# Avielstein/GRASP_LAB_SALP

Hardware: AMD Instinct MI355X
Metric: env-steps/sec at 65536 parallel envs, 1/2/4/8 MI355X; % HBM roofline (higher is better)
Workload: dtype f64

## Files before the change

grasp_lab_salp_amd/csrc/salp_device.h:

```cpp
#ifndef SALP_DEVICE_H
#define SALP_DEVICE_H

#include <hip/hip_runtime.h>
#include <stdint.h>

#include "../../include/salp.h"
#include "salp_math.h"
#include "salp_philox.h"
#include "salp_random.h"

#pragma clang fp contract(off)

static_assert(SALP_FMA, "libsalp.so is built in the product arithmetic mode (salp_math.h)");

#define SD static __device__ __forceinline__
#define SD_MEMBER __device__ __forceinline__
#define SD_HOST_DEV static __host__ __device__ __forceinline__

namespace salp {

constexpr double DT = 0.01;
constexpr double PI = 3.141592653589793;
constexpr double COS_GAMMA = 0x1.6a09e667f3bcdp-1;
constexpr double SIN_GAMMA = 0x1.6a09e667f3bccp-1;
// ... 765 lines not shown
        SF(SALP_F_AMF0 + j) = k.amf[j]; SF(SALP_F_AMRF0 + j) = k.amrf[j];
        SF(SALP_F_AMT0 + j) = k.amt[j]; SF(SALP_F_AMRT0 + j) = k.amrt[j];
    }
    h.rnd.cd = k.cd; h.rnd.dfr = k.dfr; h.rnd.dtr = k.dtr;
    h.rnd.amf0 = k.amf[0]; h.rnd.amf1 = k.amf[1]; h.rnd.amf2 = k.amf[2];
    h.rnd.amrf0 = k.amrf[0]; h.rnd.amrf1 = k.amrf[1]; h.rnd.amrf2 = k.amrf[2];
    h.rnd.amt0 = k.amt[0]; h.rnd.amt1 = k.amt[1]; h.rnd.amt2 = k.amt[2];
}

template <bool RAND = false, class ST>
SD void set_control(Hot& h, ST S, const Params& P, int64_t i, double contraction, double coast,
                    double a1, double a2, bool c32, const double* dir = nullptr) {
    set_coefficients<RAND>(h, S, P, i);
    SF(SALP_F_AVGV0) = 0.0; SF(SALP_F_AVGV1) = 0.0; SF(SALP_F_AVGV2) = 0.0;
    SF(SALP_F_AVGW0) = 0.0; SF(SALP_F_AVGW1) = 0.0; SF(SALP_F_AVGW2) = 0.0;
    h.c = contraction;
    h.coast = coast;
    h.c32 = c32;
    h.turn = nozzle_set_angles(S, P, i, a1, a2);
    if (dir) {
        h.d0 = dir[0]; h.d1 = dir[1]; h.d2 = dir[2];
    } else {
        nozzle_direction(a1, a2, &h.d0);
    }
    SF(SALP_F_CYCLE) = SF(SALP_F_CYCLE) + 1.0;
    h.ct = 0.0;
    const double sq = c32 ? (double)sqf((float)h.c) : h.c * h.c;
    h.refill = REFILL_C0 * sq + REFILL_C1 * h.c + REFILL_C2;
    h.jet = PROPUL_C0 * sq + PROPUL_C1 * h.c + PROPUL_C2;
    h.cr = h.refill > 0 ? h.c / h.refill : 0.0;
    h.rr = h.jet > 0 ? h.c / h.jet : 0.0;
    cycle_bounds(h);
}

template <class ST>
SD void cycle_prologue(const Hot& h, ST S, const Params& P, int64_t i) {
    const double total = h.b2;
    double pq0 = SF(SALP_F_PPOS0), pq1 = SF(SALP_F_PPOS1), pq2 = SF(SALP_F_PPOS2);
    double pg0 = SF(SALP_F_PANG0), pg1 = SF(SALP_F_PANG1), pg2 = SF(SALP_F_PANG2);
    SF(SALP_F_AVGV0) = (h.q0 - pq0) / total; SF(SALP_F_AVGV1) = (h.q1 - pq1) / total;
    SF(SALP_F_AVGV2) = (h.q2 - pq2) / total;
    SF(SALP_F_AVGW0) = (h.g0 - pg0) / total; SF(SALP_F_AVGW1) = (h.g1 - pg1) / total;
    SF(SALP_F_AVGW2) = (h.g2 - pg2) / total;
    SF(SALP_F_PPOS0) = h.q0; SF(SALP_F_PPOS1) = h.q1; SF(SALP_F_PPOS2) = h.q2;
    SF(SALP_F_PANG0) = h.g0; SF(SALP_F_PANG1) = h.g1; SF(SALP_F_PANG2) = h.g2;
    SF(SALP_F_PENDING) = 1.0;
}

struct StepPlan {
    float a0, a1, a2;
    double an1, an2;
    double d[3];
};
SD StepPlan plan_step(const Params& P, float a0, float a1, float a2, Cache32 c32) {
    StepPlan p;
    p.a0 = a0; p.a1 = a1; p.a2 = a2;
    const float r0 = a0 * 0.06f, r2 = a2 * (float)(PI / 2);
    nozzle_ik((double)r2, true, &p.an1, &p.an2);
    nozzle_direction(p.an1, p.an2, p.d);
    fill_cache32(P, (double)r0, c32);
    return p;
}
template <class ST>
SD void apply_step(Hot& h, ST S, const Params& P, int64_t i, const StepPlan& p) {
    SF(SALP_F_ACT0) = p.a0; SF(SALP_F_ACT1) = p.a1; SF(SALP_F_ACT2) = p.a2;
    const float r0 = p.a0 * 0.06f, r1 = p.a1 * 10.0f, r2 = p.a2 * (float)(PI / 2);
    SF(SALP_F_PREV_YAW) = SF(SALP_F_YAW);
    SF(SALP_F_YAW) = (double)r2;
    SF(SALP_F_PREV_ANGLE1) = SF(SALP_F_ANGLE1);
    SF(SALP_F_PREV_ANGLE2) = SF(SALP_F_ANGLE2);
    SF(SALP_F_ANGLE1) = p.an1;
    SF(SALP_F_ANGLE2) = p.an2;
    set_control<false>(h, S, P, i, (double)r0, (double)r1, p.an1, p.an2, true, p.d);
    cycle_prologue(h, S, P, i);
}

template <bool RAND = false, class ST>
SD void begin_step(Hot& h, ST S, const Params& P, int64_t i, float a0, float a1, float a2,
                   Cache32 c32) {
    SF(SALP_F_ACT0) = a0; SF(SALP_F_ACT1) = a1; SF(SALP_F_ACT2) = a2;
    float r0 = a0 * 0.06f, r1 = a1 * 10.0f, r2 = a2 * (float)(PI / 2);
    if (RAND && P.rand_act) {
        const float rr[3] = {r0, r1, r2};
        double ra[3];
        sr_randomize_action(P.seed, h.env_id, (uint64_t)SF(SALP_F_STEP_COUNT), rr, ra);
        nozzle_solve(S, P, i, ra[2], false);
        set_control<RAND>(h, S, P, i, ra[0], ra[1], SF(SALP_F_ANGLE1), SF(SALP_F_ANGLE2), false);
    } else {
        nozzle_solve(S, P, i, (double)r2, true);
        set_control<RAND>(h, S, P, i, (double)r0, (double)r1, SF(SALP_F_ANGLE1), SF(SALP_F_ANGLE2), true);
    }
    fill_cache32(P, h.c, c32);
    cycle_prologue(h, S, P, i);
}

template <class ST>
SD void record_state(const Hot& h, const Params& P, ST S, int64_t i, double* rec,
                     int64_t rs, bool first) {
    auto put = [&](int col, double x) { rec[(int64_t)col * rs] = x; };
    put(SALP_T_STATE, (double)h.phase);
    put(SALP_T_PW0, h.p0); put(SALP_T_PW1, h.p1); put(SALP_T_PW2, h.p2);
    put(SALP_T_V0, h.v0); put(SALP_T_V1, h.v1); put(SALP_T_V2, h.v2);
    put(SALP_T_ACC0, h.a0); put(SALP_T_ACC1, h.a1); put(SALP_T_ACC2, h.a2);
    put(SALP_T_ETA0, h.e0); put(SALP_T_ETA1, h.e1); put(SALP_T_ETA2, h.e2);
    put(SALP_T_W0, h.w0); put(SALP_T_W1, h.w1); put(SALP_T_W2, h.w2);
    put(SALP_T_ALPHA0, h.al0); put(SALP_T_ALPHA1, h.al1); put(SALP_T_ALPHA2, h.al2);
    put(SALP_T_LENGTH, h.L); put(SALP_T_WIDTH, h.W);
    const Core c = core(h.L, h.W, h.g32);
    const Shape sh = shape_of(P, c, h.L, h.W, h.g32);
    put(SALP_T_AREA0, sh.A0); put(SALP_T_AREA1, sh.A1); put(SALP_T_AREA2, sh.A1);
    put(SALP_T_VOLUME, h.V);
    put(SALP_T_MASS, h.geo.m);
    put(SALP_T_MASS_RATE, h.geo.mr);
    put(SALP_T_I0, h.geo.I0); put(SALP_T_I1, h.geo.I1); put(SALP_T_I2, h.geo.I1);
// ... 113 lines not shown
    bool done = false, trunc = false;
    if (dist < 0.2) { done = true; reward += 500.0; }
    else if (dist > 5.0) { trunc = true; reward -= 200.0; }
    if (hit) { trunc = true; reward -= 200.0; }
    if (SF(SALP_F_CYCLE) >= (double)P.max_cycles) { trunc = true; reward -= 50.0; }
    const double nlen = ep_len + 1.0;
    SF(SALP_F_EP_LEN) = nlen;
    const double ret = SF(SALP_F_EP_RETURN) + reward;
    SF(SALP_F_EP_RETURN) = ret;
    const double sa0 = SF(SALP_F_SUM_A0) + (double)(float)SF(SALP_F_ACT0);
    const double sa1 = SF(SALP_F_SUM_A1) + (double)(float)SF(SALP_F_ACT1);
    const double sa2 = SF(SALP_F_SUM_ABS_A2) + (double)fabsf(a2);
    SF(SALP_F_SUM_A0) = sa0; SF(SALP_F_SUM_A1) = sa1; SF(SALP_F_SUM_ABS_A2) = sa2;
    double sr[7];
#pragma unroll
    for (int k = 0; k < 7; ++k) {
        sr[k] = SF(SALP_F_SUM_R0 + k) + comp[k];
        SF(SALP_F_SUM_R0 + k) = sr[k];
    }
    if (info) {
        for (int k = 0; k < SALP_INFO_DIM; ++k) info[k] = 0.0;
        for (int k = 0; k < 7; ++k) info[SALP_INFO_R_TRACK + k] = comp[k];
        info[SALP_INFO_EP_RETURN] = ret;
        info[SALP_INFO_EP_LEN] = nlen;
        info[SALP_INFO_HIT_OBSTACLE] = hit ? 1.0 : 0.0;
        if (done || trunc) {
            double dd = np_norm2(px - 0.0, py - 0.0);
            info[SALP_INFO_HAS_METRICS] = 1.0;
            info[SALP_INFO_PATH_LENGTH] = path;
            info[SALP_INFO_DIRECT_DISTANCE] = dd;
            info[SALP_INFO_PATH_EFFICIENCY] = path > 0 ? dd / path : 0.0;
            info[SALP_INFO_FINAL_DISTANCE] = dist;
            info[SALP_INFO_INITIAL_DISTANCE] = SF(SALP_F_INIT_DIST);
            info[SALP_INFO_AVG_COMPRESSION] = sa0 / nlen;
            info[SALP_INFO_AVG_COAST_TIME] = sa1 / nlen;
            info[SALP_INFO_AVG_NOZZLE_ANGLE] = sa2 / nlen;
            info[SALP_INFO_AVG_VELOCITY] = svel / (nlen + 1.0);
            for (int k = 0; k < 7; ++k) info[SALP_INFO_AVG_R_TRACK + k] = sr[k] / nlen;
        }
    }
    SF(SALP_F_PREV_A2) = (double)a2;
    SF(SALP_F_PENDING) = 0.0;
    if (RAND && P.latency) {
        const double lat = sr_latency(P.seed, h.env_id, (uint64_t)SF(SALP_F_STEP_COUNT));
        set_control<RAND>(h, S, P, i, 0.0, lat, SF(SALP_F_ANGLE1), SF(SALP_F_ANGLE2), false);
    }
    out.reward = reward;
    out.terminated = done;
    out.truncated = trunc;
    out.hit = hit;
    return out;
}

SD int draw_reset(const Params& P, uint64_t env_id, uint64_t episode, float* tgt, float* obst) {
    double u0, u1;
    sp_reset_pair(P.seed, env_id, episode, 0u, &u0, &u1);
    double tx = P.x_min + (P.x_max - P.x_min) * u0, ty = P.y_min + (P.y_max - P.y_min) * u1;
    if (tx < P.x_min) tx = P.x_min;
    if (tx > P.x_max) tx = P.x_max;
    if (ty < P.y_min) ty = P.y_min;
    if (ty > P.y_max) ty = P.y_max;
    tgt[0] = (float)tx; tgt[1] = (float)ty;
    int n = 0;
    for (int k = 0; k < P.num_obstacles; ++k) {
        for (int att = 0; att < 200; ++att) {
            sp_reset_pair(P.seed, env_id, episode, (uint32_t)(1 + k * 200 + att), &u0, &u1);
            float px = (float)(P.x_min + (P.x_max - P.x_min) * u0);
            float py = (float)(P.y_min + (P.y_max - P.y_min) * u1);
            float ds = sqrtf(sm_fmaf(py, py, px * px));
            float ex = px - tgt[0], ey = py - tgt[1];
            float dtg = sqrtf(sm_fmaf(ey, ey, ex * ex));
            bool close = false;
            for (int j = 0; j < n; ++j) {
                float fx = px - obst[2 * j], fy = py - obst[2 * j + 1];
                if ((double)sqrtf(sm_fmaf(fy, fy, fx * fx)) < P.sep) close = true;
            }
            if ((double)ds > 0.5 && (double)dtg > 0.5 && !close) {
                obst[2 * n] = px; obst[2 * n + 1] = py; ++n;
                break;
            }
        }
    }
    return n;
}

template <class ST>
SD void robot_reset(Hot& h, ST S, const Params& P, int64_t i) {
    h.time = 0.0; h.ct = 0.0; h.phase = REST;
    SF(SALP_F_CYCLE) = 0.0;
    h.v0 = h.v1 = h.v2 = 0.0; h.w0 = h.w1 = h.w2 = 0.0;
    h.a0 = h.a1 = h.a2 = 0.0; h.al0 = h.al1 = h.al2 = 0.0;
    h.e0 = h.e1 = h.e2 = 0.0; h.p0 = h.p1 = h.p2 = 0.0;
    h.q0 = h.q1 = h.q2 = 0.0; h.g0 = h.g1 = h.g2 = 0.0;
    SF(SALP_F_PPOS0) = 0.0; SF(SALP_F_PPOS1) = 0.0; SF(SALP_F_PPOS2) = 0.0;
    SF(SALP_F_PANG0) = 0.0; SF(SALP_F_PANG1) = 0.0; SF(SALP_F_PANG2) = 0.0;
    {
        const Core old = core(h.L, h.W, h.g32);
        h.com = center_of_mass(P, old, water_mass(P, h.V, h.g32), h.g32);
    }
    h.comr = (h.com - h.com) / DT;
    h.coma = (h.comr - h.comr) / DT;
    h.L = P.L0; h.W = P.W0; h.g32 = false;
    const Core c0 = core(h.L, h.W, false);
    h.V = water_volume(P, c0, false);
    h.pV = h.V; h.pv32 = false;
    refresh_derived(h, P);
    h.pI0 = h.geo.I0; h.pI1 = h.geo.I1; h.pI2 = h.geo.I1;
    if (P.rand_dist) {
        SF(SALP_F_OUF0) = 0.0; SF(SALP_F_OUF1) = 0.0; SF(SALP_F_OUF2) = 0.0;
        SF(SALP_F_OUT0) = 0.0; SF(SALP_F_OUT1) = 0.0; SF(SALP_F_OUT2) = 0.0;
        h.rnd.ouf0 = 0.0; h.rnd.ouf1 = 0.0; h.rnd.out2 = 0.0;
    }
    SF(SALP_F_PENDING) = 0.0;
}

template <class ST>
SD void reset_env(Hot& h, ST S, const Params& P, int64_t i, const float* tgt,
                  const float* obst, int nob, float* obs) {
    SF(SALP_F_TARGET0) = tgt[0]; SF(SALP_F_TARGET1) = tgt[1];
#pragma unroll
    for (int k = 0; k < SALP_MAX_OBSTACLES; ++k) {
        SF(SALP_F_OBST0 + 2 * k) = k < nob ? (double)obst[2 * k] : 0.0;
        SF(SALP_F_OBST0 + 2 * k + 1) = k < nob ? (double)obst[2 * k + 1] : 0.0;
    }
    SF(SALP_F_N_OBST) = nob;
    robot_reset(h, S, P, i);
    const double d0 = h.p0 - (double)tgt[0], d1 = h.p1 - (double)tgt[1];
    const double dist = np_norm2(d0, d1);
    SF(SALP_F_PREV_DIST) = dist;
    SF(SALP_F_PREV_A2) = 0.0;
    SF(SALP_F_ACT0) = 0.0; SF(SALP_F_ACT1) = 0.0; SF(SALP_F_ACT2) = 0.0;
    SF(SALP_F_EP_LEN) = 0.0; SF(SALP_F_EP_RETURN) = 0.0; SF(SALP_F_PATH_LEN) = 0.0;
    SF(SALP_F_LAST_PX) = h.p0; SF(SALP_F_LAST_PY) = h.p1;
    SF(SALP_F_SUM_A0) = 0.0; SF(SALP_F_SUM_A1) = 0.0; SF(SALP_F_SUM_ABS_A2) = 0.0;
    SF(SALP_F_SUM_VEL) = np_norm2(0.0, 0.0);
    SF(SALP_F_INIT_DIST) = dist;
#pragma unroll
    for (int k = 0; k < 7; ++k) SF(SALP_F_SUM_R0 + k) = 0.0;
    SF(SALP_F_EPISODE) = SF(SALP_F_EPISODE) + 1.0;
    SF(SALP_F_PENDING) = 0.0;
    if (obs) {
        Rot R = rot_zyx(h.e0, h.e1, h.e2);
        observation(h, R, S, P, i, obs);
    }
}

template <class ST>
SD void reset_env_philox(Hot& h, ST S, const Params& P, int64_t i, float* obs) {
    float tgt[2], obst[2 * SALP_MAX_OBSTACLES];
    int nob = draw_reset(P, (uint64_t)(P.env_offset + i), (uint64_t)SF(SALP_F_EPISODE), tgt, obst);
    reset_env(h, S, P, i, tgt, obst, nob, obs);
}

template <bool RAND>
SD void load_cold(ColdRegs<RAND>& C, double* S, const Params& P, int64_t i) {
    C.g = S + i;
    C.n = P.n;
    if (!SALP_COLD_BLOCK) {
#pragma unroll
        for (int f = 0; f < SALP_NUM_FIELDS; ++f)
            if (is_cached<RAND>(f)) C.v[f] = S[(size_t)f * (size_t)P.n + (size_t)i];
        return;
    }
    const double2* blk = reinterpret_cast<const double2*>(S + P.cold_off + (size_t)i * COLD_SLOTS);
    double v[kLayout.n_cold + 1];
#pragma unroll
    for (int k = 0; k < (kLayout.n_cold + 1) / 2; ++k) {
        const double2 x = blk[k];
        v[2 * k] = x.x;
        v[2 * k + 1] = x.y;
    }
#pragma unroll
    for (int f = 0; f < SALP_NUM_FIELDS; ++f) {
        if (kLayout.slot[f] >= 0) C.v[f] = v[kLayout.slot[f]];
        else if (is_cached<RAND>(f)) C.v[f] = S[(size_t)kLayout.row[f] * (size_t)P.n + (size_t)i];
    }
}
template <bool RAND>
SD void store_cold(const ColdRegs<RAND>& C, double* S, const Params& P, int64_t i) {
    if (!SALP_COLD_BLOCK) {
#pragma unroll
        for (int f = 0; f < SALP_NUM_FIELDS; ++f)
            if (is_cached<RAND>(f)) S[(size_t)f * (size_t)P.n + (size_t)i] = C.v[f];
        return;
    }
    double v[kLayout.n_cold + 1];
#pragma unroll
    for (int f = 0; f < SALP_NUM_FIELDS; ++f) {
        if (kLayout.slot[f] >= 0) v[kLayout.slot[f]] = C.v[f];
        else if (is_cached<RAND>(f)) S[(size_t)kLayout.row[f] * (size_t)P.n + (size_t)i] = C.v[f];
    }
    v[kLayout.n_cold] = 0.0;
    double2* blk = reinterpret_cast<double2*>(S + P.cold_off + (size_t)i * COLD_SLOTS);
#pragma unroll
    for (int k = 0; k < (kLayout.n_cold + 1) / 2; ++k) blk[k] = make_double2(v[2 * k], v[2 * k + 1]);
}

constexpr int SPILL_N = 63;
constexpr int SPILL_D0 = 43;
struct SpillSlot {
    double* p;
    int stride = LANES;
    SD_MEMBER double& operator[](int k) const { return p[k * stride]; }
};
template <bool RAND>
SD void spill(const Hot& h, SpillSlot s) {
    const Hot::Rnd& r = h.rnd;
    const double v[SPILL_N] = {
        h.v0, h.v1, h.v2, h.w0, h.w1, h.w2, h.a0, h.a1, h.a2, h.al0, h.al1, h.al2,
        h.e0, h.e1, h.e2, h.p0, h.p1, h.p2, h.q0, h.q1, h.q2, h.g0, h.g1, h.g2,
        h.L, h.W, h.V, h.pV, h.com, h.comr, h.coma, h.pI0, h.pI1, h.pI2, h.ct, h.time,
        h.refill, h.jet, h.coast, h.c, h.cr, h.rr, h.turn, h.d0, h.d1, h.d2,
        (double)(h.phase | (h.g32 ? 4 : 0) | (h.pv32 ? 8 : 0) | (h.c32 ? 16 : 0)),
        RAND ? r.cd : h.sp, RAND ? r.dfr : h.cp, RAND ? r.dtr : h.st, RAND ? r.amf0 : h.cth,
        RAND ? r.amf1 : h.geo.m, RAND ? r.amf2 : h.geo.mr, RAND ? r.amrf0 : h.geo.I0,
        RAND ? r.amrf1 : h.geo.I1, RAND ? r.amrf2 : h.geo.kc0, RAND ? r.amt0 : h.geo.kc1,
        RAND ? r.amt1 : h.geo.ra0, RAND ? r.amt2 : h.geo.ra1, RAND ? r.ouf0 : h.geo.dimx,
        RAND ? r.ouf1 : h.geo.dimy, RAND ? r.out2 : h.geo.speed, RAND ? r.tick : h.geo.rx};
#pragma unroll
    for (int k = 0; k < SPILL_N; ++k) s[k] = v[k];
}
template <bool RAND>
SD void unspill(Hot& h, SpillSlot s, const Params& P, uint64_t env_id) {
    double v[SPILL_N];
#pragma unroll
    for (int k = 0; k < SPILL_N; ++k) v[k] = s[k];
    h.v0 = v[0]; h.v1 = v[1]; h.v2 = v[2]; h.w0 = v[3]; h.w1 = v[4]; h.w2 = v[5];
    h.a0 = v[6]; h.a1 = v[7]; h.a2 = v[8]; h.al0 = v[9]; h.al1 = v[10]; h.al2 = v[11];
    h.e0 = v[12]; h.e1 = v[13]; h.e2 = v[14]; h.p0 = v[15]; h.p1 = v[16]; h.p2 = v[17];
    h.q0 = v[18]; h.q1 = v[19]; h.q2 = v[20]; h.g0 = v[21]; h.g1 = v[22]; h.g2 = v[23];
    h.L = v[24]; h.W = v[25]; h.V = v[26]; h.pV = v[27]; h.com = v[28]; h.comr = v[29]; h.coma = v[30];
    h.pI0 = v[31]; h.pI1 = v[32]; h.pI2 = v[33]; h.ct = v[34]; h.time = v[35];
    h.refill = v[36]; h.jet = v[37]; h.coast = v[38]; h.c = v[39]; h.cr = v[40]; h.rr = v[41];
    h.turn = v[42]; h.d0 = v[43]; h.d1 = v[44]; h.d2 = v[45];
    const int fl = (int)v[46];
    h.phase = fl & 3; h.g32 = (fl & 4) != 0; h.pv32 = (fl & 8) != 0; h.c32 = (fl & 16) != 0;
    h.env_id = env_id;
    if (RAND) {
        Hot::Rnd& r = h.rnd;
        r.cd = v[47]; r.dfr = v[48]; r.dtr = v[49]; r.amf0 = v[50]; r.amf1 = v[51]; r.amf2 = v[52];
        r.amrf0 = v[53]; r.amrf1 = v[54]; r.amrf2 = v[55]; r.amt0 = v[56]; r.amt1 = v[57];
        r.amt2 = v[58]; r.ouf0 = v[59]; r.ouf1 = v[60]; r.out2 = v[61]; r.tick = v[62];
        refresh_derived(h, P);
    } else {
        h.sp = v[47]; h.cp = v[48]; h.st = v[49]; h.cth = v[50];
        h.geo.m = v[51]; h.geo.mr = v[52]; h.geo.I0 = v[53]; h.geo.I1 = v[54]; h.geo.kc0 = v[55];
        h.geo.kc1 = v[56]; h.geo.ra0 = v[57]; h.geo.ra1 = v[58]; h.geo.dimx = v[59]; h.geo.dimy = v[60];
        h.geo.speed = v[61]; h.geo.rx = v[62];
        geo_recips(h.geo);
    }
    cycle_bounds(h);
}
// ... 44 lines not shown
```

grasp_lab_salp_amd/csrc/salp_kernels.hip:

```cpp
#include <hip/hip_runtime.h>

#include <cmath>
#include <cstdio>
#include <cstdlib>
#include <cstring>
#include <string>

#include "salp_device.h"
#include "salp_pair.h"
#include "salp_tanh.h"

using salp::Hot;
using salp::Params;

#define SF(f) salp::sref(S, P, i, (f))

namespace {

constexpr int kBlock = 256;
constexpr int kMaxTicksPerCycle = 1 << 16;
constexpr int64_t kSortMinEnvs = 1024;

static_assert(kBlock == salp::LANES, "LDS cache stride is the workgroup size");

// ... 560 lines not shown
    for (int j = 0; j < NW - 1; ++j) {
        const int c = __popcll(m[j]);
        if (k < c) {
            w = m[j];
            base = 64 * j;
            break;
        }
        k -= c;
        base = 64 * (j + 1);
    }
    int pos = 0;
#pragma unroll
    for (int half = 32; half > 0; half >>= 1) {
        const uint64_t lo = w & ((1ull << half) - 1ull);
        const int c = __popcll(lo);
        if (k >= c) {
            k -= c;
            w >>= half;
            pos += half;
        } else {
            w = lo;
        }
    }
    return base + pos;
}

__device__ __forceinline__ bool unsteady(const Hot& h, const Params& P, bool active) {
    return active && h.ct < h.b2 && !salp::next_tick_steady(h, P);
}

template <bool RAND, bool POL>
__device__ __forceinline__ bool lane_boundary(const RolloutArgs& a, salp::SpillSlot sp, int64_t i, bool& pending,
                                              bool& active, int64_t& steps, double* c32p) {
    const uint64_t env_id = (uint64_t)(a.P.env_offset + i);
    salp::ColdRegs<RAND> C;
    salp::load_cold<RAND>(C, a.S, a.P, i);
    Hot hb;
    salp::unspill<RAND>(hb, sp, a.P, env_id);
    rollout_boundary<RAND, POL>(hb, &C, a.P, i, env_id, pending, active, steps, a.max_steps, a.B,
                                a.reward_sum, a.R, salp::Cache32{c32p});
    salp::store_cold<RAND>(C, a.S, a.P, i);
    salp::spill<RAND>(hb, sp);
    return unsteady(hb, a.P, active);
}
template <bool RAND, bool POL>
__device__ __noinline__ bool lane_boundary_call(const RolloutArgs* a, double* spp, int64_t i, bool* pending,
                                                bool* active, int64_t* steps, double* c32p) {
    return lane_boundary<RAND, POL>(*a, salp::SpillSlot{spp}, i, *pending, *active, *steps, c32p);
}

#ifndef SALP_ROLLOUT_PROF
#define SALP_ROLLOUT_PROF 0
#endif
enum { RP_BOUNDARY, RP_FULL, RP_STEADY, RP_SETTLED, RP_BARRIER, RP_RESEAT, RP_B_LOAD, RP_B_FINISH, RP_B_PLAN,
       RP_B_JOIN, RP_N };
__device__ unsigned long long g_roll_prof[2][RP_N];
struct RollProf {
    unsigned long long cyc[RP_N] = {}, its[RP_N] = {};
    unsigned long long t = 0;
    __device__ __forceinline__ void start() {
        if (SALP_ROLLOUT_PROF) t = __builtin_amdgcn_s_memtime();
    }
    __device__ __forceinline__ void lap(int part, int64_t iterations = 0) {
        if (SALP_ROLLOUT_PROF) {
            const unsigned long long now = __builtin_amdgcn_s_memtime();
            cyc[part] += now - t;
            its[part] += (unsigned long long)iterations;
            t = now;
        }
    }
    __device__ __forceinline__ void flush() {
        if (SALP_ROLLOUT_PROF && (threadIdx.x & 63) == 0)
            for (int k = 0; k < RP_N; ++k) {
                atomicAdd(&g_roll_prof[0][k], cyc[k]);
                atomicAdd(&g_roll_prof[1][k], its[k]);
            }
    }
};

#if SALP_ROLLOUT_RESEAT
typedef __attribute__((address_space(3))) double LdsDouble;
enum { TK_TICKING = 1, TK_UNSTEADY = 2 };
__device__ __forceinline__ RolloutArgs args_of(uint64_t kernarg) {
    const uint32_t lo = __builtin_amdgcn_readfirstlane((uint32_t)kernarg);
    const uint32_t hi = __builtin_amdgcn_readfirstlane((uint32_t)(kernarg >> 32));
    return args_at((KernargWords)(((uint64_t)hi << 32) | lo));
}
__device__ __forceinline__ uint32_t tick_flags(const Hot& h, const Params& P, bool active) {
    return (uint32_t)((h.ct < h.b2 ? TK_TICKING : 0) | (unsteady(h, P, active) ? TK_UNSTEADY : 0));
}
#if SALP_ROLLOUT_PROF
#define ROLL_PROF_PARAM , RollProf& prof
#define ROLL_PROF_ARG , prof
#else
#define ROLL_PROF_PARAM
#define ROLL_PROF_ARG
#endif
template <bool RAND>
[[clang::not_tail_called]] __device__ __noinline__ uint32_t wave_ticks(uint64_t kernarg, LdsDouble* spp,
                                                                       LdsDouble* c32p, int64_t i,
                                                                       uint32_t active ROLL_PROF_PARAM) {
#if !SALP_ROLLOUT_PROF
    RollProf prof;
#endif
    const salp::SpillSlot sp{(double*)spp};
    const salp::Cache32 c32{(double*)c32p};
    const RolloutArgs A = args_of(kernarg);
    const int32_t chunk = A.chunk, steady_q8 = A.steady_q8;
    Hot h;
    salp::unspill<RAND>(h, sp, A.P, (uint64_t)(A.P.env_offset + i));
    if (!active) h.b2 = -INFINITY;
    prof.lap(RP_RESEAT);
    const Params PV = salp::pin_params(A.P);
    int32_t k = 0;
    for (; k < chunk; ++k) {
        if (__all(!(h.ct < h.b2) || salp::next_tick_steady(h, PV))) break;
        if (h.ct < h.b2) salp::tick<false, RAND, true>(h, PV, c32);
    }
    prof.lap(RP_FULL, k);
    const int32_t ks = (int32_t)(((int64_t)(chunk - k) * steady_q8) >> 8);
    int32_t j = 0;
    while (j < ks) {
        bool settled = true;
        if (h.ct < h.b2) settled = salp::tick<false, RAND, true, true>(h, PV, c32);
        ++j;
        if (__all(settled)) break;
    }
    prof.lap(RP_STEADY, j);
    const int32_t j0 = j;
    for (; j < ks; ++j)
        if (h.ct < h.b2) salp::tick<false, RAND, true, true, true>(h, PV, c32);
    prof.lap(RP_SETTLED, j - j0);
    const uint32_t tk = tick_flags(h, args_of(kernarg).P, active != 0);
    salp::spill<RAND>(h, sp);
    return tk;
}

enum { FL_PENDING = 1, FL_ACTIVE = 2, FL_TICKING = 4 };
constexpr int kRoleJobs = kBlock / 2;
struct RoleLds {
    double* spill;
    double* cache32;
    int64_t* steps;
    uint8_t* flags;
    const int16_t* slot_of;
    uint64_t* mask;
    uint64_t* amask;
};

template <class ST>
__device__ __forceinline__ bool role_finish(Hot& h, ST S, const Params& P, int64_t i, bool& pending, bool& active,
                                            int64_t& steps, int64_t max_steps, const SalpRolloutBuffers& B,
                                            double* reward_sum, float* o, bool& have_o) {
    const bool fin = active && pending && !(h.ct < h.b2);
    if (fin) {
        SF(SALP_F_STEP_COUNT) = SF(SALP_F_STEP_COUNT) + 1.0;
        salp::StepOut r = salp::finish_step<false>(h, S, P, i, o, nullptr);
        const bool reset = r.terminated || r.truncated;
        if (B.capacity > 0) {
            const size_t slot = (size_t)(steps % B.capacity);
            const size_t row = slot * (size_t)P.n + (size_t)i;
            if (B.obs)
                for (int k = 0; k < P.obs_dim; ++k) B.obs[row * P.obs_dim + k] = o[k];
            if (B.actions) {
                B.actions[row * 3 + 0] = (float)SF(SALP_F_ACT0);
                B.actions[row * 3 + 1] = (float)SF(SALP_F_ACT1);
                B.actions[row * 3 + 2] = (float)SF(SALP_F_ACT2);
            }
            if (B.rewards) B.rewards[row] = (float)r.reward;
            if (B.dones) B.dones[row] = (uint8_t)((r.terminated ? 1 : 0) | (r.truncated ? 2 : 0));
        }
        if (reward_sum) reward_sum[i] += r.reward;
        ++steps;
        pending = false;
        if (reset) salp::reset_env_philox(h, S, P, i, B.obs_before ? o : nullptr);
        have_o = true;
        if (max_steps > 0 && steps >= max_steps) active = false;
    }
    const bool beg = active && !pending;
    if (beg && B.obs_before) {
        if (!have_o) {
            const salp::Rot Rt = salp::rot_zyx(h.e0, h.e1, h.e2);
            salp::observation(h, Rt, S, P, i, o);
            have_o = true;
        }
        if (B.capacity > 0) {
            const size_t row = (size_t)(steps % B.capacity) * (size_t)P.n + (size_t)i;
            for (int k = 0; k < P.obs_dim; ++k) B.obs_before[row * P.obs_dim + k] = o[k];
        }
    }
    return beg;
}

__device__ __forceinline__ uint64_t pack_floats(float lo, float hi) {
    return (uint64_t)__float_as_uint(lo) | ((uint64_t)__float_as_uint(hi) << 32);
}

__device__ __forceinline__ void role_boundary(const RoleLds L, const int b, const int lane, const int64_t base,
                                              const bool need, RollProf& prof) {
    __shared__ uint64_t s_need[2][kBlock / 64];
    __shared__ uint32_t s_again[2][2][4];
    __shared__ uint64_t s_plan[4][kRoleJobs];
    const uint64_t nb = __ballot(need);
    if ((lane & 63) == 0) s_need[b][lane >> 6] = nb;
    if (lane < 8) (&s_again[b][0][0])[lane] = 0u;
    prof.lap(RP_BOUNDARY);
    __syncthreads();
    prof.lap(RP_BARRIER);
    uint64_t nm[kBlock / 64];
    int n_jobs = 0;
#pragma unroll
    for (int w = 0; w < kBlock / 64; ++w) {
        nm[w] = s_need[b][w];
        n_jobs += __popcll(nm[w]);
    }
    const bool fin_role = lane < kRoleJobs;
    const int jr = lane & (kRoleJobs - 1);
    for (int p = 0; p * kRoleJobs < n_jobs; ++p) {
        const int j = p * kRoleJobs + jr;
        const bool has = j < n_jobs;
        int jl = 0, js = 0;
        if (has) {
            jl = nth_set_lane(nm, j);
            js = L.slot_of[jl];
        }
        const int64_t i = base + js;
        const salp::SpillSlot sp{L.spill + js};
        salp::ColdRegs<false> C;
        Hot hb;
        float o[SALP_OBS_DIM_MAX];
        bool have_o = false, pending = false, active = false, live = fin_role && has;
        int64_t steps = 0;
        bool go = false;
        double sc = 0.0;
        prof.lap(RP_BOUNDARY);
        if (has) {
            const RolloutArgs a = fresh_args();
            const int fl = L.flags[js];
            if (fin_role) {
                salp::load_cold<false>(C, a.S, a.P, i);
                salp::unspill<false>(hb, sp, a.P, (uint64_t)(a.P.env_offset + i));
                pending = (fl & FL_PENDING) != 0;
                active = (fl & FL_ACTIVE) != 0;
                steps = L.steps[js];
            } else {
                const bool fin = (fl & FL_ACTIVE) && (fl & FL_PENDING) && !(fl & FL_TICKING);
                const int64_t st = L.steps[js] + (fin ? 1 : 0);
                go = !(fin && a.max_steps > 0 && st >= a.max_steps);
                sc = salp::sref((const double*)a.S, a.P, i, SALP_F_STEP_COUNT) + (fin ? 1.0 : 0.0);
            }
        }
        prof.lap(RP_B_LOAD);
        for (int r = 0;; ++r) {
            bool beg = false;
            if (fin_role) {
                if (live) {
                    const RolloutArgs a = fresh_args();
                    beg = role_finish(hb, &C, a.P, i, pending, active, steps, a.max_steps, a.B, a.reward_sum, o,
                                      have_o);
                }
                prof.lap(RP_B_FINISH);
            } else {
                if (go) {
                    const RolloutArgs a = fresh_args();
                    float act[3];
                    sp_action(a.P.seed, (uint64_t)(a.P.env_offset + i), (uint64_t)sc, act);
                    const salp::StepPlan pl =
                        salp::plan_step(a.P, act[0], act[1], act[2], salp::Cache32{L.cache32 + js});
                    s_plan[0][jr] = pack_floats(pl.a0, pl.a1);
                    s_plan[1][jr] = pack_floats(pl.a2, 0.0f);
                    s_plan[2][jr] = (uint64_t)__double_as_longlong(pl.an1);
                    s_plan[3][jr] = (uint64_t)__double_as_longlong(pl.an2);
#pragma unroll
                    for (int k = 0; k < 3; ++k) sp[salp::SPILL_D0 + k] = pl.d[k];
                }
                prof.lap(RP_B_PLAN);
            }
            prof.lap(RP_BOUNDARY);
            __syncthreads();
            prof.lap(RP_BARRIER);
            if (live) {
                const RolloutArgs a = fresh_args();
                if (beg) {
                    salp::StepPlan pl;
                    const uint64_t w0 = s_plan[0][jr], w1 = s_plan[1][jr];
                    pl.a0 = __uint_as_float((uint32_t)w0);
                    pl.a1 = __uint_as_float((uint32_t)(w0 >> 32));
                    pl.a2 = __uint_as_float((uint32_t)w1);
                    pl.an1 = __longlong_as_double((long long)s_plan[2][jr]);
                    pl.an2 = __longlong_as_double((long long)s_plan[3][jr]);
#pragma unroll
                    for (int k = 0; k < 3; ++k) pl.d[k] = sp[salp::SPILL_D0 + k];
                    salp::apply_step(hb, &C, a.P, i, pl);
                    pending = true;
                }
                const bool again = r < 3 && active && pending && !(hb.ct < hb.b2);
                if (again) {
                    s_again[b][p][r] = 1u;
                    s_plan[0][jr] =
                        (uint64_t)__double_as_longlong(salp::sref(&C, a.P, i, SALP_F_STEP_COUNT) + 1.0);
                    s_plan[1][jr] = (a.max_steps > 0 && steps + 1 >= a.max_steps) ? 0u : 1u;
                } else {
                    s_plan[1][jr] = 0u;
                    salp::store_cold<false>(C, a.S, a.P, i);
                    salp::spill<false>(hb, sp);
                    L.flags[js] = (uint8_t)((pending ? FL_PENDING : 0) | (active ? FL_ACTIVE : 0));
                    L.steps[js] = steps;
                    const uint64_t bit = 1ull << (jl & 63);
                    if (unsteady(hb, a.P, active)) atomicOr((unsigned long long*)&L.mask[jl >> 6], bit);
                    if (!active) atomicAnd((unsigned long long*)&L.amask[jl >> 6], ~bit);
                    live = false;
                }
            }
            prof.lap(RP_B_JOIN);
            __syncthreads();
            prof.lap(RP_BARRIER);
            if (r == 3 || !s_again[b][p][r]) break;
            go = false;
            if (!fin_role && has && s_plan[1][jr] != 0u) {
                go = true;
                sc = __longlong_as_double((long long)s_plan[0][jr]);
            }
        }
    }
}

template <bool RAND, bool POL>
__global__ __launch_bounds__(kBlock) void k_rollout(RolloutArgs A) {
    double* const S = A.S;
    const Params& P = A.P;
    const int64_t base = (int64_t)blockIdx.x * blockDim.x;
    const int lane = (int)threadIdx.x;
    constexpr bool kRoles = !RAND && !POL;
    __shared__ double s_cache32[salp::C32_N * salp::LANES];
    __shared__ double s_spill[salp::SPILL_N * salp::LANES];
    __shared__ int64_t s_steps[kBlock];
    __shared__ uint8_t s_flags[kBlock];
    __shared__ int16_t s_slot[2][kBlock];
    __shared__ uint64_t s_mask[2][kBlock / 64];
    __shared__ uint64_t s_amask[2][kBlock / 64];
    int s = lane;
    int64_t i = base + s;
    bool pending = false, active = false;
    int64_t steps = 0;
    uint32_t tk;
    {
        Hot h{};
        if (i < P.n) {
            pending = !A.fresh && SF(SALP_F_PENDING) != 0.0;
            steps = A.B.steps_done ? A.B.steps_done[i] : 0;
            active = !(A.max_steps > 0 && steps >= A.max_steps);
            salp::load_hot<RAND>(h, S, P, i);
            salp::resume_cycle(h, S, P, i);
            salp::fill_cache32(P, h.c, salp::Cache32{s_cache32 + s});
        }
        if (!active) h.b2 = -INFINITY;
        tk = tick_flags(h, P, active);
        salp::spill<RAND>(h, salp::SpillSlot{s_spill + s});
    }
    bool all_done = false;
    RollProf prof;
    prof.start();
    for (int64_t c = 0;; ++c) {
        const bool last = c == A.n_chunks || all_done;
        const salp::SpillSlot sp{s_spill + s};
        const bool need = active && (!pending || !(tk & TK_TICKING));
        bool uns = (tk & TK_UNSTEADY) != 0;
        if constexpr (kRoles) {
            const int b = (int)(c & 1);
            s_steps[s] = steps;
            s_flags[s] = (uint8_t)((pending ? FL_PENDING : 0) | (active ? FL_ACTIVE : 0) |
                                   ((tk & TK_TICKING) ? FL_TICKING : 0));
            s_slot[b][lane] = (int16_t)s;
            const uint64_t ballot = __ballot(uns && !need);
            const uint64_t aballot = __ballot(active);
            if ((lane & 63) == 0) {
                s_mask[b][lane >> 6] = ballot;
                s_amask[b][lane >> 6] = aballot;
// ... 1836 lines not shown
```

Measured before the change: 77.76 million.

## Split boundary work across four wave roles: finish, observe, plan, reset draw

Boundary handling in the rollout kernel now uses four 64-lane waves, each with its own role, instead of two halves split between finish and plan. Wave 0 does the core finish, reward and rows. Wave 1 computes observations from spilled state and fills the cache32 table. Wave 2 draws actions and does nozzle IK and direction. Wave 3 pre-draws reset targets and obstacles into LDS. The aim is to take serial work (observation, reset draw, cache fill) off the finishing lanes, at the cost of more shared memory, duplicated action sampling and recomputed observations.

```diff
diff --git a/grasp_lab_salp_amd/csrc/salp_device.h b/grasp_lab_salp_amd/csrc/salp_device.h
--- a/grasp_lab_salp_amd/csrc/salp_device.h
+++ b/grasp_lab_salp_amd/csrc/salp_device.h
@@ -841,14 +841,14 @@
     double an1, an2;
     double d[3];
 };
-SD StepPlan plan_step(const Params& P, float a0, float a1, float a2, Cache32 c32) {
-    StepPlan p;
-    p.a0 = a0; p.a1 = a1; p.a2 = a2;
-    const float r0 = a0 * 0.06f, r2 = a2 * (float)(PI / 2);
+SD void plan_angles(StepPlan& p) {
+    const float r2 = p.a2 * (float)(PI / 2);
     nozzle_ik((double)r2, true, &p.an1, &p.an2);
-    nozzle_direction(p.an1, p.an2, p.d);
+}
+SD void plan_direction(StepPlan& p) { nozzle_direction(p.an1, p.an2, p.d); }
+SD void plan_cache(const Params& P, float a0, Cache32 c32) {
+    const float r0 = a0 * 0.06f;
     fill_cache32(P, (double)r0, c32);
-    return p;
 }
 template <class ST>
 SD void apply_step(Hot& h, ST S, const Params& P, int64_t i, const StepPlan& p) {
@@ -1068,6 +1068,87 @@
     return out;
 }
 
+template <class ST>
+SD StepOut finish_core(Hot& h, ST S, const Params& P, int64_t i) {
+    StepOut out;
+    const Rot R = rot_zyx(h.e0, h.e1, h.e2);
+    double vw[3];
+    world_frame(h.e0, h.e1, h.e2, h.v0, h.v1, h.v2, vw, sm_poly());
+    const double px = h.p0, py = h.p1;
+    double path = SF(SALP_F_PATH_LEN) + np_norm2(px - SF(SALP_F_LAST_PX), py - SF(SALP_F_LAST_PY));
+    SF(SALP_F_PATH_LEN) = path;
+    SF(SALP_F_LAST_PX) = px; SF(SALP_F_LAST_PY) = py;
+    double svel = SF(SALP_F_SUM_VEL) + np_norm2(vw[0], vw[1]);
+    SF(SALP_F_SUM_VEL) = svel;
+    const double tx = SF(SALP_F_TARGET0), ty = SF(SALP_F_TARGET1);
+    const double dx = px - tx, dy = py - ty;
+    const double dist = np_norm2(dx, dy);
+    double comp[7];
+    comp[0] = (-dist + SF(SALP_F_PREV_DIST)) * 100;
+    SF(SALP_F_PREV_DIST) = dist;
+    double b0, b1;
+    rot_body_xy(R, dx, dy, &b0, &b1);
+    comp[1] = -0.5 * fabs(sm_atan2(-b1, -b0));
+    const float a2 = (float)SF(SALP_F_ACT2);
+    const double ep_len = SF(SALP_F_EP_LEN);
+    if (ep_len == 0.0) {
+        double ch = (double)a2 - SF(SALP_F_PREV_A2);
+        comp[2] = -1.0 * (ch * ch);
+    } else {
+        float ch = a2 - (float)SF(SALP_F_PREV_A2);
+        comp[2] = (double)(-(ch * ch));
+    }
+    comp[3] = -10.0 * fabs(SF(SALP_F_AVGW2));
+    comp[4] = -0.1;
+    comp[5] = -100.0 * fabs(SF(SALP_F_AVGV1));
+    comp[6] = 0.0;
+    const int nob = (int)SF(SALP_F_N_OBST);
+    double md = 0.0;
+#pragma unroll
+    for (int k = 0; k < SALP_MAX_OBSTACLES; ++k) {
+        if (k >= nob) break;
+        double d = np_norm2(px - SF(SALP_F_OBST0 + 2 * k), py - SF(SALP_F_OBST0 + 2 * k + 1));
+        if (k == 0 || d < md) md = d;
+    }
+    if (nob > 0) {
+        double danger = 2.0 * P.obstacle_radius;
+        if (md < danger) comp[6] = -1.0 * (1.0 - md / danger);
+    }
+    double reward = comp[0] + comp[1] + comp[2] + comp[3] + comp[4] + comp[5] + comp[6];
+    bool l32;
+    double Lc, Wc;
+    body_lw(P, h.phase, h.ct, h.refill, h.mx, h.c, h.cr, h.rr, h.c32, &Lc, &Wc, &l32);
+    double thr = l32 ? (double)((float)P.obstacle_radius + (float)Lc / 2.0f)
+                     : P.obstacle_radius + Lc / 2;
+    bool hit = false;
+#pragma unroll
+    for (int k = 0; k < SALP_MAX_OBSTACLES; ++k) {
+        if (k >= nob) break;
+        double d = np_norm2(px - SF(SALP_F_OBST0 + 2 * k), py - SF(SALP_F_OBST0 + 2 * k + 1));
+        if (d < thr) hit = true;
+    }
+    bool done = false, trunc = false;
+    if (dist < 0.2) { done = true; reward += 500.0; }
+    else if (dist > 5.0) { trunc = true; reward -= 200.0; }
+    if (hit) { trunc = true; reward -= 200.0; }
+    if (SF(SALP_F_CYCLE) >= (double)P.max_cycles) { trunc = true; reward -= 50.0; }
+    SF(SALP_F_EP_LEN) = ep_len + 1.0;
+    SF(SALP_F_EP_RETURN) = SF(SALP_F_EP_RETURN) + reward;
+    const double sa0 = SF(SALP_F_SUM_A0) + (double)(float)SF(SALP_F_ACT0);
+    const double sa1 = SF(SALP_F_SUM_A1) + (double)(float)SF(SALP_F_ACT1);
+    const double sa2 = SF(SALP_F_SUM_ABS_A2) + (double)fabsf(a2);
+    SF(SALP_F_SUM_A0) = sa0; SF(SALP_F_SUM_A1) = sa1; SF(SALP_F_SUM_ABS_A2) = sa2;
+#pragma unroll
+    for (int k = 0; k < 7; ++k) SF(SALP_F_SUM_R0 + k) = SF(SALP_F_SUM_R0 + k) + comp[k];
+    SF(SALP_F_PREV_A2) = (double)a2;
+    SF(SALP_F_PENDING) = 0.0;
+    out.reward = reward;
+    out.terminated = done;
+    out.truncated = trunc;
+    out.hit = hit;
+    return out;
+}
+
 SD int draw_reset(const Params& P, uint64_t env_id, uint64_t episode, float* tgt, float* obst) {
     double u0, u1;
     sp_reset_pair(P.seed, env_id, episode, 0u, &u0, &u1);
@@ -1161,6 +1242,23 @@
     }
 }
 
+SD void reset_observation(const Params& P, const float* tgt, const float* obst, int nob, float* obs) {
+    Hot h;
+    h.p0 = h.p1 = 0.0; h.v0 = h.v1 = 0.0; h.w2 = 0.0;
+    ColdRegs<false> C;
+    ColdRegs<false>* S = &C;
+    const int64_t i = 0;
+    SF(SALP_F_TARGET0) = tgt[0]; SF(SALP_F_TARGET1) = tgt[1];
+#pragma unroll
+    for (int k = 0; k < SALP_MAX_OBSTACLES; ++k) {
+        SF(SALP_F_OBST0 + 2 * k) = k < nob ? (double)obst[2 * k] : 0.0;
+        SF(SALP_F_OBST0 + 2 * k + 1) = k < nob ? (double)obst[2 * k + 1] : 0.0;
+    }
+    SF(SALP_F_N_OBST) = nob;
+    const Rot R = rot_zyx(0.0, 0.0, 0.0);
+    observation(h, R, S, P, i, obs);
+}
+
 template <class ST>
 SD void reset_env_philox(Hot& h, ST S, const Params& P, int64_t i, float* obs) {
     float tgt[2], obst[2 * SALP_MAX_OBSTACLES];
@@ -1214,6 +1312,7 @@
 
 constexpr int SPILL_N = 63;
 constexpr int SPILL_D0 = 43;
+constexpr int SPILL_V0 = 0, SPILL_W2 = 5, SPILL_E0 = 12, SPILL_P0 = 15;
 struct SpillSlot {
     double* p;
     int stride = LANES;
diff --git a/grasp_lab_salp_amd/csrc/salp_kernels.hip b/grasp_lab_salp_amd/csrc/salp_kernels.hip
--- a/grasp_lab_salp_amd/csrc/salp_kernels.hip
+++ b/grasp_lab_salp_amd/csrc/salp_kernels.hip
@@ -636,8 +636,9 @@
 #ifndef SALP_ROLLOUT_PROF
 #define SALP_ROLLOUT_PROF 0
 #endif
-enum { RP_BOUNDARY, RP_FULL, RP_STEADY, RP_SETTLED, RP_BARRIER, RP_RESEAT, RP_B_LOAD, RP_B_FINISH, RP_B_PLAN,
-       RP_B_JOIN, RP_N };
+enum { RP_BOUNDARY, RP_FULL, RP_STEADY, RP_SETTLED, RP_BARRIER, RP_RESEAT, RP_B_LOAD, RP_B_FINISH, RP_B_ROWS,
+       RP_B_RESET, RP_B_JOIN, RP_O_OBS, RP_O_BEFORE, RP_P_ACTION, RP_P_IK, RP_P_DIR, RP_C_ACTION, RP_C_CACHE,
+       RP_C_DRAW, RP_N };
 __device__ unsigned long long g_roll_prof[2][RP_N];
 struct RollProf {
     unsigned long long cyc[RP_N] = {}, its[RP_N] = {};
@@ -721,7 +722,11 @@
 }
 
 enum { FL_PENDING = 1, FL_ACTIVE = 2, FL_TICKING = 4 };
-constexpr int kRoleJobs = kBlock / 2;
+enum { NOTE_NONE, NOTE_SAME, NOTE_RESET };
+constexpr int kRoleJobs = 64;
+constexpr int kRolePasses = kBlock / kRoleJobs;
+constexpr int kDrawWords = 3 + 2 * SALP_MAX_OBSTACLES;
+static_assert(kBlock == 4 * 64, "role_boundary: four waves, one role each");
 struct RoleLds {
     double* spill;
     double* cache32;
@@ -732,62 +737,27 @@
     uint64_t* amask;
 };
 
-template <class ST>
-__device__ __forceinline__ bool role_finish(Hot& h, ST S, const Params& P, int64_t i, bool& pending, bool& active,
-                                            int64_t& steps, int64_t max_steps, const SalpRolloutBuffers& B,
-                                            double* reward_sum, float* o, bool& have_o) {
-    const bool fin = active && pending && !(h.ct < h.b2);
-    if (fin) {
-        SF(SALP_F_STEP_COUNT) = SF(SALP_F_STEP_COUNT) + 1.0;
-        salp::StepOut r = salp::finish_step<false>(h, S, P, i, o, nullptr);
-        const bool reset = r.terminated || r.truncated;
-        if (B.capacity > 0) {
-            const size_t slot = (size_t)(steps % B.capacity);
-            const size_t row = slot * (size_t)P.n + (size_t)i;
-            if (B.obs)
-                for (int k = 0; k < P.obs_dim; ++k) B.obs[row * P.obs_dim + k] = o[k];
-            if (B.actions) {
-                B.actions[row * 3 + 0] = (float)SF(SALP_F_ACT0);
-                B.actions[row * 3 + 1] = (float)SF(SALP_F_ACT1);
-                B.actions[row * 3 + 2] = (float)SF(SALP_F_ACT2);
-            }
-            if (B.rewards) B.rewards[row] = (float)r.reward;
-            if (B.dones) B.dones[row] = (uint8_t)((r.terminated ? 1 : 0) | (r.truncated ? 2 : 0));
-        }
-        if (reward_sum) reward_sum[i] += r.reward;
-        ++steps;
-        pending = false;
-        if (reset) salp::reset_env_philox(h, S, P, i, B.obs_before ? o : nullptr);
-        have_o = true;
-        if (max_steps > 0 && steps >= max_steps) active = false;
-    }
-    const bool beg = active && !pending;
-    if (beg && B.obs_before) {
-        if (!have_o) {
-            const salp::Rot Rt = salp::rot_zyx(h.e0, h.e1, h.e2);
-            salp::observation(h, Rt, S, P, i, o);
-            have_o = true;
-        }
-        if (B.capacity > 0) {
-            const size_t row = (size_t)(steps % B.capacity) * (size_t)P.n + (size_t)i;
-            for (int k = 0; k < P.obs_dim; ++k) B.obs_before[row * P.obs_dim + k] = o[k];
-        }
-    }
-    return beg;
-}
-
 __device__ __forceinline__ uint64_t pack_floats(float lo, float hi) {
     return (uint64_t)__float_as_uint(lo) | ((uint64_t)__float_as_uint(hi) << 32);
+}
+
+__device__ __forceinline__ void store_obs_row(float* row, const float* o, int obs_dim) {
+#pragma unroll
+    for (int k = 0; k < SALP_OBS_DIM_MAX; ++k)
+        if (k < obs_dim) row[k] = o[k];
 }
 
 __device__ __forceinline__ void role_boundary(const RoleLds L, const int b, const int lane, const int64_t base,
                                               const bool need, RollProf& prof) {
     __shared__ uint64_t s_need[2][kBlock / 64];
-    __shared__ uint32_t s_again[2][2][4];
+    __shared__ uint32_t s_again[2][kRolePasses][4];
     __shared__ uint64_t s_plan[4][kRoleJobs];
+    __shared__ float s_draw[kRoleJobs][kDrawWords];
+    __shared__ uint8_t s_note[kRoleJobs];
+    __shared__ uint8_t s_live[kRoleJobs];
     const uint64_t nb = __ballot(need);
     if ((lane & 63) == 0) s_need[b][lane >> 6] = nb;
-    if (lane < 8) (&s_again[b][0][0])[lane] = 0u;
+    if (lane < kRolePasses * 4) (&s_again[b][0][0])[lane] = 0u;
     prof.lap(RP_BOUNDARY);
     __syncthreads();
     prof.lap(RP_BARRIER);
@@ -798,7 +768,7 @@
         nm[w] = s_need[b][w];
         n_jobs += __popcll(nm[w]);
     }
-    const bool fin_role = lane < kRoleJobs;
+    const int role = __builtin_amdgcn_readfirstlane(lane >> 6);
     const int jr = lane & (kRoleJobs - 1);
     for (int p = 0; p * kRoleJobs < n_jobs; ++p) {
         const int j = p * kRoleJobs + jr;
@@ -812,45 +782,119 @@
         const salp::SpillSlot sp{L.spill + js};
         salp::ColdRegs<false> C;
         Hot hb;
+        bool pending = false, active = false;
+        int64_t steps = 0;
         float o[SALP_OBS_DIM_MAX];
-        bool have_o = false, pending = false, active = false, live = fin_role && has;
-        int64_t steps = 0;
-        bool go = false;
-        double sc = 0.0;
+        bool live = has;
         prof.lap(RP_BOUNDARY);
-        if (has) {
+        if (role == 0 && has) {
             const RolloutArgs a = fresh_args();
             const int fl = L.flags[js];
-            if (fin_role) {
-                salp::load_cold<false>(C, a.S, a.P, i);
-                salp::unspill<false>(hb, sp, a.P, (uint64_t)(a.P.env_offset + i));
-                pending = (fl & FL_PENDING) != 0;
-                active = (fl & FL_ACTIVE) != 0;
-                steps = L.steps[js];
-            } else {
-                const bool fin = (fl & FL_ACTIVE) && (fl & FL_PENDING) && !(fl & FL_TICKING);
-                const int64_t st = L.steps[js] + (fin ? 1 : 0);
-                go = !(fin && a.max_steps > 0 && st >= a.max_steps);
-                sc = salp::sref((const double*)a.S, a.P, i, SALP_F_STEP_COUNT) + (fin ? 1.0 : 0.0);
-            }
+            salp::load_cold<false>(C, a.S, a.P, i);
+            salp::unspill<false>(hb, sp, a.P, (uint64_t)(a.P.env_offset + i));
+            pending = (fl & FL_PENDING) != 0;
+            active = (fl & FL_ACTIVE) != 0;
+            steps = L.steps[js];
         }
         prof.lap(RP_B_LOAD);
         for (int r = 0;; ++r) {
-            bool beg = false;
-            if (fin_role) {
+            bool fin = false, go = false;
+            int64_t st = 0;
+            if (role != 0 && live) {
+                const RolloutArgs a = fresh_args();
+                const int fl = L.flags[js];
+                fin = (fl & FL_ACTIVE) && (fl & FL_PENDING) && !(fl & FL_TICKING);
+                st = L.steps[js];
+                go = !(fin && a.max_steps > 0 && st + 1 >= a.max_steps);
+            }
+            bool beg = false, rst = false;
+            if (role == 0) {
+                const bool fin0 = live && active && pending && !(hb.ct < hb.b2);
+                salp::StepOut so{};
+                if (fin0) {
+                    const RolloutArgs a = fresh_args();
+                    salp::sref(&C, a.P, i, SALP_F_STEP_COUNT) = salp::sref(&C, a.P, i, SALP_F_STEP_COUNT) + 1.0;
+                    so = salp::finish_core(hb, &C, a.P, i);
+                }
+                prof.lap(RP_B_FINISH);
+                if (fin0) {
+                    const RolloutArgs a = fresh_args();
+                    rst = so.terminated || so.truncated;
+                    if (a.B.capacity > 0) {
+                        const size_t row = (size_t)(steps % a.B.capacity) * (size_t)a.P.n + (size_t)i;
+                        if (a.B.actions) {
+                            a.B.actions[row * 3 + 0] = (float)salp::sref(&C, a.P, i, SALP_F_ACT0);
+                            a.B.actions[row * 3 + 1] = (float)salp::sref(&C, a.P, i, SALP_F_ACT1);
+                            a.B.actions[row * 3 + 2] = (float)salp::sref(&C, a.P, i, SALP_F_ACT2);
+                        }
+                        if (a.B.rewards) a.B.rewards[row] = (float)so.reward;
+                        if (a.B.dones)
+                            a.B.dones[row] = (uint8_t)((so.terminated ? 1 : 0) | (so.truncated ? 2 : 0));
+                    }
+                    if (a.reward_sum) a.reward_sum[i] += so.reward;
+                    ++steps;
+                    pending = false;
+                    if (a.max_steps > 0 && steps >= a.max_steps) active = false;
+                }
+                if (live) {
+                    beg = active && !pending;
+                    s_note[jr] = beg ? (rst ? NOTE_RESET : NOTE_SAME) : NOTE_NONE;
+                }
+                prof.lap(RP_B_ROWS);
+            } else if (role == 1) {
                 if (live) {
                     const RolloutArgs a = fresh_args();
-                    beg = role_finish(hb, &C, a.P, i, pending, active, steps, a.max_steps, a.B, a.reward_sum, o,
-                                      have_o);
+                    if (fin ? (a.B.obs != nullptr || a.B.obs_before != nullptr) : a.B.obs_before != nullptr) {
+                        Hot ho;
+                        ho.v0 = sp[salp::SPILL_V0];
+                        ho.v1 = sp[salp::SPILL_V0 + 1];
+                        ho.w2 = sp[salp::SPILL_W2];
+                        ho.e0 = sp[salp::SPILL_E0];
+                        ho.e1 = sp[salp::SPILL_E0 + 1];
+                        ho.e2 = sp[salp::SPILL_E0 + 2];
+                        ho.p0 = sp[salp::SPILL_P0];
+                        ho.p1 = sp[salp::SPILL_P0 + 1];
+                        const salp::Rot Rt = salp::rot_zyx(ho.e0, ho.e1, ho.e2);
+                        salp::observation(ho, Rt, (const double*)a.S, a.P, i, o);
+                        if (fin && a.B.obs && a.B.capacity > 0) {
+                            const size_t row = (size_t)(st % a.B.capacity) * (size_t)a.P.n + (size_t)i;
+                            store_obs_row(a.B.obs + row * a.P.obs_dim, o, a.P.obs_dim);
+                        }
+                    }
                 }
-                prof.lap(RP_B_FINISH);
-            } else {
+                prof.lap(RP_O_OBS);
+                float a0 = 0.0f;
                 if (go) {
                     const RolloutArgs a = fresh_args();
+                    const double sc =
+                        salp::sref((const double*)a.S, a.P, i, SALP_F_STEP_COUNT) + (fin ? 1.0 : 0.0);
                     float act[3];
                     sp_action(a.P.seed, (uint64_t)(a.P.env_offset + i), (uint64_t)sc, act);
-                    const salp::StepPlan pl =
-                        salp::plan_step(a.P, act[0], act[1], act[2], salp::Cache32{L.cache32 + js});
+                    a0 = act[0];
+                }
+                prof.lap(RP_C_ACTION);
+                if (go) {
+                    const RolloutArgs a = fresh_args();
+                    salp::plan_cache(a.P, a0, salp::Cache32{L.cache32 + js});
+                }
+                prof.lap(RP_C_CACHE);
+            } else if (role == 2) {
+                salp::StepPlan pl{};
+                if (go) {
+                    const RolloutArgs a = fresh_args();
+                    const double sc =
+                        salp::sref((const double*)a.S, a.P, i, SALP_F_STEP_COUNT) + (fin ? 1.0 : 0.0);
+                    float act[3];
+                    sp_action(a.P.seed, (uint64_t)(a.P.env_offset + i), (uint64_t)sc, act);
+                    pl.a0 = act[0];
+                    pl.a1 = act[1];
+                    pl.a2 = act[2];
+                }
+                prof.lap(RP_P_ACTION);
+                if (go) salp::plan_angles(pl);
+                prof.lap(RP_P_IK);
+                if (go) {
+                    salp::plan_direction(pl);
                     s_plan[0][jr] = pack_floats(pl.a0, pl.a1);
                     s_plan[1][jr] = pack_floats(pl.a2, 0.0f);
                     s_plan[2][jr] = (uint64_t)__double_as_longlong(pl.an1);
@@ -858,56 +902,82 @@
 #pragma unroll
                     for (int k = 0; k < 3; ++k) sp[salp::SPILL_D0 + k] = pl.d[k];
                 }
-                prof.lap(RP_B_PLAN);
+                prof.lap(RP_P_DIR);
+            } else {
+                if (fin) {
+                    const RolloutArgs a = fresh_args();
+                    const uint64_t episode = (uint64_t)salp::sref((const double*)a.S, a.P, i, SALP_F_EPISODE);
+                    float* const rec = s_draw[jr];
+                    rec[2] = (float)salp::draw_reset(a.P, (uint64_t)(a.P.env_offset + i), episode, rec, rec + 3);
+                }
+                prof.lap(RP_C_DRAW);
             }
             prof.lap(RP_BOUNDARY);
             __syncthreads();
             prof.lap(RP_BARRIER);
-            if (live) {
-                const RolloutArgs a = fresh_args();
-                if (beg) {
-                    salp::StepPlan pl;
-                    const uint64_t w0 = s_plan[0][jr], w1 = s_plan[1][jr];
-                    pl.a0 = __uint_as_float((uint32_t)w0);
-                    pl.a1 = __uint_as_float((uint32_t)(w0 >> 32));
-                    pl.a2 = __uint_as_float((uint32_t)w1);
-                    pl.an1 = __longlong_as_double((long long)s_plan[2][jr]);
-                    pl.an2 = __longlong_as_double((long long)s_plan[3][jr]);
+            if (role == 0) {
+                if (live && rst) {
+                    const RolloutArgs a = fresh_args();
+                    const float* const rec = s_draw[jr];
+                    salp::reset_env(hb, &C, a.P, i, rec, rec + 3, (int)rec[2], nullptr);
+                }
+                prof.lap(RP_B_RESET);
+                if (live) {
+                    const RolloutArgs a = fresh_args();
+                    if (beg) {
+                        salp::StepPlan pl;
+                        const uint64_t w0 = s_plan[0][jr], w1 = s_plan[1][jr];
+                        pl.a0 = __uint_as_float((uint32_t)w0);
+                        pl.a1 = __uint_as_float((uint32_t)(w0 >> 32));
+                        pl.a2 = __uint_as_float((uint32_t)w1);
+                        pl.an1 = __longlong_as_double((long long)s_plan[2][jr]);
+                        pl.an2 = __longlong_as_double((long long)s_plan[3][jr]);
 #pragma unroll
-                    for (int k = 0; k < 3; ++k) pl.d[k] = sp[salp::SPILL_D0 + k];
-                    salp::apply_step(hb, &C, a.P, i, pl);
-                    pending = true;
-                }
-                const bool again = r < 3 && active && pending && !(hb.ct < hb.b2);
-                if (again) {
-                    s_again[b][p][r] = 1u;
-                    s_plan[0][jr] =
-                        (uint64_t)__double_as_longlong(salp::sref(&C, a.P, i, SALP_F_STEP_COUNT) + 1.0);
-                    s_plan[1][jr] = (a.max_steps > 0 && steps + 1 >= a.max_steps) ? 0u : 1u;
-                } else {
-                    s_plan[1][jr] = 0u;
+                        for (int k = 0; k < 3; ++k) pl.d[k] = sp[salp::SPILL_D0 + k];
+                        salp::apply_step(hb, &C, a.P, i, pl);
+                        pending = true;
+                    }
+                    const bool again = r < 3 && active && pending && !(hb.ct < hb.b2);
                     salp::store_cold<false>(C, a.S, a.P, i);
                     salp::spill<false>(hb, sp);
                     L.flags[js] = (uint8_t)((pending ? FL_PENDING : 0) | (active ? FL_ACTIVE : 0));
                     L.steps[js] = steps;
-                    const uint64_t bit = 1ull << (jl & 63);
-                    if (unsteady(hb, a.P, active)) atomicOr((unsigned long long*)&L.mask[jl >> 6], bit);
-                    if (!active) atomicAnd((unsigned long long*)&L.amask[jl >> 6], ~bit);
-                    live = false;
+                    s_live[jr] = again ? 1 : 0;
+                    if (again) {
+                        s_again[b][p][r] = 1u;
+                    } else {
+                        const uint64_t bit = 1ull << (jl & 63);
+                        if (unsteady(hb, a.P, active)) atomicOr((unsigned long long*)&L.mask[jl >> 6], bit);
+                        if (!active) atomicAnd((unsigned long long*)&L.amask[jl >> 6], ~bit);
+                        live = false;
+                    }
                 }
+                prof.lap(RP_B_JOIN);
+            } else if (role == 1) {
+                if (live) {
+                    const RolloutArgs a = fresh_args();
+                    const int note = fin ? s_note[jr] : NOTE_SAME;
+                    if (note != NOTE_NONE && a.B.obs_before && a.B.capacity > 0) {
+                        if (note == NOTE_RESET) {
+                            const float* const rec = s_draw[jr];
+                            salp::reset_observation(a.P, rec, rec + 3, (int)rec[2], o);
+                        }
+                        const size_t row =
+                            (size_t)((st + (fin ? 1 : 0)) % a.B.capacity) * (size_t)a.P.n + (size_t)i;
+                        store_obs_row(a.B.obs_before + row * a.P.obs_dim, o, a.P.obs_dim);
+                    }
+                }
+                prof.lap(RP_O_BEFORE);
             }
-            prof.lap(RP_B_JOIN);
+            prof.lap(RP_BOUNDARY);
             __syncthreads();
             prof.lap(RP_BARRIER);
             if (r == 3 || !s_again[b][p][r]) break;
-            go = false;
-            if (!fin_role && has && s_plan[1][jr] != 0u) {
-                go = true;
-                sc = __longlong_as_double((long long)s_plan[0][jr]);
-            }
-        }
-    }
-}
+            if (role != 0) live = has && s_live[jr] != 0;
+        }
+    }
+}
+
 
 template <bool RAND, bool POL>
 __global__ __launch_bounds__(kBlock) void k_rollout(RolloutArgs A) {
```

After: 79.75 million (median of 6 runs). 1.03x the previous value.
